# Kolkir/mono_slam_framework

Measured on AMD Instinct MI355X. Metric: frame-pairs/sec (extract+match), higher is better.
Workload: dtype u8; 1 GPU; ORB extract+match, 1280x720 pairs, 1024 pairs/GPU/step resident in HBM, ratio 0.60; pairs_per_gpu=1024, width=1280, height=720, synth_mode=0, overflow_pairs=0, ranks=1, rccl_ranks=0

## Files before the change

mono_slam_framework_amd/csrc/orb_kernels.hip:

```cpp
#include <type_traits>
#include "orb_pipeline.h"

#include <math.h>
#include <stdlib.h>
#include <string.h>

#include "orb_blur_tiles.h"
#include "orb_pattern.h"

namespace msf {

constexpr int SW = TW + 2, SH = TH + 2;
constexpr int kTileCandCap = TW * TH / 4;
constexpr int kTileY0 = kEdge;

constexpr uint32_t kStatusOverflow = 1u;

__constant__ __attribute__((aligned(16))) signed char c_pattern[1024];
__constant__ uint32_t c_disc[2 * kDiscTasks];

__device__ __forceinline__ __amdgpu_buffer_rsrc_t uniform_rsrc(const void* p, uint32_t bytes) {
  const unsigned long long v = (unsigned long long)p;
  const uint32_t lo = (uint32_t)__builtin_amdgcn_readfirstlane((int)(uint32_t)v);
  const uint32_t hi = (uint32_t)__builtin_amdgcn_readfirstlane((int)(uint32_t)(v >> 32));
// ... 1331 lines not shown
                                             int resize_mask, int test_stall_frame, int finish, uint32_t* s1_cnt,
                                             uint4* s1) {
  __shared__ StreamSmem sm;
  const WalkUnit u = walk_unit(g, l_lo, l_hi, n_frames, finish, blockIdx.x);
  if (u.kind == kWalkNone) return;
  const int l = u.level, fi = u.frame, ts = u.strip;
  if (u.kind == kWalkThreshold) {
    if (fi == test_stall_frame && l == 3) return;
    tau_unit(*reinterpret_cast<TauSmem*>(&sm), g, src, pyr, tau, tau_first, redo_cnt, redo_list, qstat, status, abort_word,
             force_tau, predict_pct, chain, l, fi);
    return;
  }
  if (u.kind == kWalkFinish) {
    finish_unit(*reinterpret_cast<FinishSmem*>(&sm), g, src, pyr, tau, tau_first, qstat, cand_cnt, cand_key, cand_sc, cmap,
                redo_cnt, redo_list, s1_cnt, s1, status, abort_word, l, fi);
    return;
  }
  if ((resize_mask >> l) & 1)
    walk_strip<true>(sm, g, src, pyr, tab, qstat, cand_cnt, cand_key, cand_sc, cmap, status, abort_word, margin_pct, dyn, chain, l, fi, ts);
  else
    walk_strip<false>(sm, g, src, pyr, tab, qstat, cand_cnt, cand_key, cand_sc, cmap, status, abort_word, margin_pct, dyn, chain, l, fi, ts);
}

__global__ __launch_bounds__(64) void k_fast_check(OrbGeometry g, int n_frames, uint32_t* tau, uint32_t* tau_first,
                                                   uint32_t* cand_cnt, const uint8_t* cand_sc, const uint2* cmap,
                                                   uint32_t* redo_cnt, uint32_t* redo_list, const uint32_t* qstat) {
  const int fi = blockIdx.x / kOrbLevels, l = blockIdx.x - fi * kOrbLevels, lane = threadIdx.x;
  if (fi >= n_frames || l >= g.nlevels) return;
  const int idx = fi * kOrbLevels + l;
  if (qstat[(size_t)idx * kQStat + kQFin] != 0u) return;
  if (tau[idx] <= (uint32_t)kFastT) return;
  const uint32_t T = max(tau[idx], qstat[(size_t)idx * kQStat + kQTau]);
  const OrbLevelInfo L = g.lv[l];
  const uint2 cm = cmap[idx];
  const bool over = cand_cnt[idx] > cm.y;
  const uint32_t n = min(cand_cnt[idx], cm.y);
  const uint8_t* scs = cand_sc + cm.x;
  const uint32_t found = count_scores_from(scs, n, T, lane);
  if (lane == 0) {
    if (over || found < 2u * (uint32_t)L.quota) {
      tau[idx] = kFastT;
      cand_cnt[idx] = 0;
      redo_list[atomicAdd(redo_cnt, 1u)] = (uint32_t)(fi * kOrbLevels + l);
    } else {
      tau[idx] = T;
      tau_first[idx] = T;
    }
  }
}

__global__ __launch_bounds__(kFastThreads) void k_fast_redo(OrbGeometry g, FrameSrc src, const uint8_t* pyr,
                                                            const uint32_t* __restrict__ redo_cnt,
                                                            const uint32_t* __restrict__ redo_list, int max_tiles,
                                                            uint32_t* cand_cnt, uint32_t* cand_key, uint8_t* cand_sc,
                                                            const uint2* cmap, uint32_t* hist, const uint32_t* emit_thr) {
  __shared__ FastSmem sm;
  const uint32_t n = *redo_cnt;
  const unsigned long long units = (unsigned long long)n * (unsigned)max_tiles;
  const unsigned long long per_xcd = (units + 7ull) >> 3;
  const unsigned long long u_begin = (blockIdx.x & 7u) * per_xcd;
  const unsigned long long u_end = u_begin + per_xcd < units ? u_begin + per_xcd : units;
  for (unsigned long long u = u_begin + (blockIdx.x >> 3); u < u_end; u += (gridDim.x >> 3)) {
    const uint32_t item = redo_list[u / (unsigned)max_tiles];
    const int t = (int)(u % (unsigned)max_tiles);
    const int fi = (int)(item / kOrbLevels), l = (int)(item % kOrbLevels);
    if (t >= g.lv[l].tiles_x * g.lv[l].tiles_y) continue;
    uint32_t emit_min = 0u;
    if (emit_thr) {
      emit_min = emit_thr[item];
      if (emit_min > 255u) continue;
    }
    fast_tile(g, src, pyr, fi, l, t, kFastT, cand_cnt, cand_key, cand_sc, cmap, sm, hist, emit_min);
    __syncthreads();
  }
}

__global__ __launch_bounds__(64) void k_redo_thr(OrbGeometry g, const uint32_t* __restrict__ redo_cnt,
                                                 const uint32_t* __restrict__ redo_list, const uint2* cmap, uint32_t* hist,
                                                 uint32_t* emit_thr) {
  const uint32_t n = *redo_cnt;
  const int lane = threadIdx.x;
  for (uint32_t q = blockIdx.x; q < n; q += gridDim.x) {
    const uint32_t item = redo_list[q];
    const int l = (int)(item % kOrbLevels);
    const int idx = (int)item;
    uint4* const hl = reinterpret_cast<uint4*>(hist + (size_t)idx * 256u);
    const uint4 hv = hl[lane];
    hl[lane] = make_uint4(0u, 0u, 0u, 0u);
    const uint32_t keep = 2u * (uint32_t)g.lv[l].quota;
    uint32_t above = hv.x + hv.y + hv.z + hv.w;
#pragma unroll
    for (int o = 1; o < 64; o <<= 1) {
      const uint32_t up = __shfl_down(above, o);
      if (lane + o < 64) above += up;
    }
    const uint32_t total = __shfl(above, 0);
    above -= hv.x + hv.y + hv.z + hv.w;
    const uint32_t c3 = above + hv.w, c2 = c3 + hv.z, c1 = c2 + hv.y, c0 = c1 + hv.x;
    const int mine = c3 >= keep ? 4 * lane + 3 : c2 >= keep ? 4 * lane + 2 : c1 >= keep ? 4 * lane + 1 : c0 >= keep ? 4 * lane : -1;
    const unsigned long long ok = __ballot(mine >= 0);
    uint32_t thr = 0;
    if (total > keep && total > cmap[idx].y) {
      thr = 256;
      if (keep > 0 && ok) thr = (uint32_t)__shfl(mine, 63 - __builtin_clzll(ok));
    }
    if (lane == 0) emit_thr[idx] = thr;
  }
}

__global__ __launch_bounds__(256) void k_thr_harris(OrbGeometry g, FrameSrc src, const uint8_t* pyr,
                                                    const uint32_t* cand_cnt, const uint32_t* cand_key,
                                                    const uint8_t* cand_sc, const uint2* cmap,
                                                    uint32_t* s1_cnt, uint4* s1, uint32_t* status, int do_harris,
                                                    const uint32_t* fin) {
  __shared__ Stage1Smem S;
  const int l = blockIdx.x, fi = blockIdx.y, tid = threadIdx.x;
  if (l >= g.nlevels) return;
  const int idx = fi * kOrbLevels + l;
  const int slot = src.slot0 + fi;
  if (fin && fin[(size_t)idx * kQStat + kQFin] != 0u) return;
  uint32_t n = cand_cnt[idx];
  const uint2 cm = cmap[idx];
  if (n > cm.y) {
    if (tid == 0) atomicOr(&status[slot], kStatusOverflow);
    n = cm.y;
  }
  stage1_from_list<9>(S, g, src, pyr, l, fi, n, cm, cand_key, cand_sc, s1_cnt, s1, status, do_harris, tid, blockDim.x);
}

__global__ __launch_bounds__(256) void k_harris_flat(OrbGeometry g, FrameSrc src, const uint8_t* pyr, HarrisUnits hw,
                                                     const uint32_t* __restrict__ s1_cnt, uint4* s1,
                                                     const uint32_t* fin) {
  const int fi = blockIdx.y, lane = threadIdx.x & 63;
  const int u = blockIdx.x * 4 + (threadIdx.x >> 6);
  if (u >= hw.base[g.nlevels]) return;
  int l = 0;
#pragma unroll
  for (int i = 1; i < kOrbLevels; i++)
    if (i < g.nlevels && u >= hw.base[i]) l = i;
  if (fin && fin[(size_t)(fi * kOrbLevels + l) * kQStat + kQFin] != 0u) return;
  const OrbLevelInfo L = g.lv[l];
  const uint32_t kept = min(s1_cnt[fi * kOrbLevels + l], (uint32_t)kS1Cap);
  uint4* out = s1 + (long long)fi * g.s1_total + L.s1_off;
  int pitch;
  const uint8_t* img = level_ptr(g, src, pyr, fi, l, &pitch);
  const uint32_t step = 64u * (uint32_t)hw.n[l];
  for (uint32_t i = 64u * (uint32_t)(u - hw.base[l]) + lane; i < kept; i += step) {
    const uint32_t key = out[i].x;
    out[i].y = __float_as_uint(harris_at(img, pitch, key & 0xFFFF, key >> 16));
  }
}

constexpr int kSelCap = kKpCap;
__global__ __launch_bounds__(256) void k_select(OrbGeometry g, int slot0, const uint32_t* s1_cnt, const uint4* s1,
                                                msf_keypoint* kp, uint32_t* kp_cnt, uint32_t* status) {
  __shared__ uint4 kept[kSelCap];
  constexpr int kRespCap = 4096;
  __shared__ __attribute__((aligned(16))) float resp[kRespCap];
  __shared__ __attribute__((aligned(16))) uint32_t keys[kSelCap];
  __shared__ uint32_t nkept;
  const int fi = blockIdx.x, tid = threadIdx.x;
  const int slot = slot0 + fi;
  msf_keypoint* out = kp + (long long)slot * kKpCap;
  uint32_t base = 0;
  bool overflow = false;
  for (int l = 0; l < g.nlevels; l++) {
    const OrbLevelInfo L = g.lv[l];
    const uint32_t n = s1_cnt[fi * kOrbLevels + l];
    const uint4* in = s1 + (long long)fi * g.s1_total + L.s1_off;
    const uint32_t keep = (uint32_t)L.quota;
    if (tid == 0) nkept = 0;
    const bool staged = n > keep && n <= (uint32_t)kRespCap;
    const uint32_t n4 = (n + 3) >> 2;
    if (staged)
      for (uint32_t i = tid; i < 4 * n4; i += 256) resp[i] = i < n ? __uint_as_float(in[i].y) : -INFINITY;
    __syncthreads();
    for (uint32_t i = tid; i < n; i += 256) {
      const uint4 e = in[i];
      bool k = true;
      if (n > keep) {
        const float v = __uint_as_float(e.y);
        uint32_t greater = 0;
        if (staged) {
          const float4* r4 = reinterpret_cast<const float4*>(resp);
          for (uint32_t j = 0; j < n4; j++) {
            const float4 r = r4[j];
            greater += (uint32_t)(r.x > v) + (uint32_t)(r.y > v) + (uint32_t)(r.z > v) + (uint32_t)(r.w > v);
          }
        } else {
          for (uint32_t j = 0; j < n; j++) greater += (__uint_as_float(in[j].y) > v) ? 1u : 0u;
        }
        k = greater < keep;
      }
      if (k) {
        const uint32_t q = atomicAdd(&nkept, 1u);
        if (q < (uint32_t)kSelCap) kept[q] = e;
      }
    }
    __syncthreads();
    uint32_t m = nkept;
    if (m > (uint32_t)kSelCap) { overflow = true; m = kSelCap; }
    if (base + m > (uint32_t)kKpCap) { overflow = true; m = kKpCap - base; }
    const uint32_t m4 = (m + 3) >> 2;
    for (uint32_t i = tid; i < 4 * m4; i += 256) keys[i] = i < m ? kept[i].x : 0xFFFFFFFFu;
    __syncthreads();
    for (uint32_t i = tid; i < m; i += 256) {
      const uint4 e = kept[i];
      uint32_t rank = 0;
      const uint4* k4 = reinterpret_cast<const uint4*>(keys);
      for (uint32_t j = 0; j < m4; j++) {
        const uint4 kk = k4[j];
        rank += (uint32_t)(kk.x < e.x) + (uint32_t)(kk.y < e.x) + (uint32_t)(kk.z < e.x) + (uint32_t)(kk.w < e.x);
      }
      msf_keypoint k;
      k.lx = e.x & 0xFFFF;
      k.ly = e.x >> 16;
      k.x = (float)k.lx * L.scale;
      k.y = (float)k.ly * L.scale;
      k.response = __uint_as_float(e.y);
      k.angle = -1.f;
      k.octave = l;
      k.fast_score = (int)e.z;
      out[base + rank] = k;
    }
    base += m;
    __syncthreads();
  }
  if (tid == 0) {
    kp_cnt[slot] = base;
    if (overflow) atomicOr(&status[slot], kStatusOverflow);
  }
}

__device__ __forceinline__ float fast_atan2_deg(float y, float x) {
  const float k = (float)(180.0 / 3.14159265358979323846);
  const float p1 = 0.9997878412794807f * k, p3 = -0.3258083974640975f * k, p5 = 0.1555786518463281f * k,
              p7 = -0.04432655554792128f * k;
  const float ax = fabsf(x), ay = fabsf(y);
  float a, c, c2;
  if (ax >= ay) {
    c = ay / (ax + (float)2.2204460492503131e-16);
    c2 = c * c;
    a = (((p7 * c2 + p5) * c2 + p3) * c2 + p1) * c;
  } else {
    c = ax / (ay + (float)2.2204460492503131e-16);
    c2 = c * c;
    a = 90.f - (((p7 * c2 + p5) * c2 + p3) * c2 + p1) * c;
  }
  if (x < 0) a = 180.f - a;
  if (y < 0) a = 360.f - a;
  return a;
}

__device__ __forceinline__ void det_sincosf(float t, float* s, float* c) {
  const double x = (double)t;
  const int k = (int)(x * 6.36619772367581382433e-01 + 0.5);
  const double kd = (double)k;
  const double r = (x - kd * 1.57079632673412561417e+00) - kd * 6.07710050650619224932e-11;
  const double z = r * r;
  double p = 1.58969099521155010221e-10;
  p = p * z + -2.50507602534068634195e-08;
  p = p * z + 2.75573137070700676789e-06;
  p = p * z + -1.98412698298579493134e-04;
  p = p * z + 8.33333333332248946124e-03;
  p = p * z + -1.66666666666666324348e-01;
  const double sr = r + (r * z) * p;
  double q = -1.13596475577881948265e-11;
  q = q * z + 2.08757232129817482790e-09;
  q = q * z + -2.75573143513906633035e-07;
  q = q * z + 2.48015872894767294178e-05;
  q = q * z + -1.38888888888741095749e-03;
  q = q * z + 4.16666666666666019037e-02;
  const double cr = (1.0 - 0.5 * z) + (z * z) * q;
  double sv, cv;
  switch (k & 3) {
    case 0: sv = sr; cv = cr; break;
    case 1: sv = cr; cv = -sr; break;
    case 2: sv = -sr; cv = -cr; break;
    default: sv = -cr; cv = sr; break;
  }
  *s = (float)sv;
  *c = (float)cv;
}

constexpr int PR = 22;
constexpr int PD = 2 * PR + 1;
constexpr int PP = blur_tiles::kRawPitch;
constexpr int HP = blur_tiles::kHbCols;
constexpr int HC = blur_tiles::kHbPitch;
static_assert(PD == blur_tiles::kRawRows && PD * (PP / 4) == blur_tiles::kFetchLoads * blur_tiles::kFetchLanes, "patch fetch");
typedef int v4i_t __attribute__((ext_vector_type(4)));

template <bool HALF_UP, bool SUM256>
__global__ __launch_bounds__(256) void k_describe(OrbGeometry g, FrameSrc src, const uint8_t* pyr,
                                                  msf_keypoint* kp, const uint32_t* kp_cnt, uint8_t* desc) {
  __shared__ __attribute__((aligned(16))) uint8_t raw_s[4][blur_tiles::kRawBytes];
  __shared__ __attribute__((aligned(16))) uint16_t hb_s[4][blur_tiles::kHbEntries];
  __shared__ uint32_t disc_s[2 * kDiscTasks];
  __shared__ __attribute__((aligned(16))) int pat_s[256];
  int fi = blockIdx.y, part = blockIdx.x;
  if (gridDim.x == 8 && (fi | 7) < (int)gridDim.y) {
    part = fi & 7;
    fi = (fi & ~7) | (int)blockIdx.x;
  }
  const int slot = src.slot0 + fi;
  const int wave = __builtin_amdgcn_readfirstlane((int)(threadIdx.x >> 6)), lane = threadIdx.x & 63;
  for (int i = threadIdx.x; i < 2 * kDiscTasks; i += 256) disc_s[i] = c_disc[i];
  pat_s[threadIdx.x] = reinterpret_cast<const int*>(c_pattern)[threadIdx.x];
  __shared__ unsigned long long lvl_base_s[kOrbLevels];
  __shared__ int lvl_pitch_s[kOrbLevels];
  if (threadIdx.x < kOrbLevels) {
    int pt = 0;
    const uint8_t* bp = level_ptr(g, src, pyr, fi, threadIdx.x < g.nlevels ? (int)threadIdx.x : 0, &pt);
    lvl_base_s[threadIdx.x] = (unsigned long long)bp;
    lvl_pitch_s[threadIdx.x] = pt;
  }
  __syncthreads();
  const uint32_t count = min(kp_cnt[slot], (uint32_t)kKpCap);
  uint8_t* raw = raw_s[wave];
  uint16_t* hb = hb_s[wave];
  uint32_t* raw32 = reinterpret_cast<uint32_t*>(raw);
  constexpr int NPL = blur_tiles::kFetchLoads;
  const uint32_t kstride = gridDim.x * 4;
  uint32_t k = (uint32_t)part * 4 + wave;
  uint32_t pre[NPL];
  auto meta = [&](uint32_t k_) -> uint3 {
    if (k_ >= count) return make_uint3(0u, 0u, 0u);
    const msf_keypoint* Kp = kp + (long long)slot * kKpCap + k_;
    return make_uint3((uint32_t)Kp->octave, (uint32_t)Kp->lx, (uint32_t)Kp->ly);
  };
  const int fl = blur_tiles::fetch_lane(lane);
  const uint32_t fetch_row = (uint32_t)blur_tiles::fetch_row(lane), fetch_x4 = 4u * (uint32_t)blur_tiles::fetch_dword(lane);
  auto issue = [&](uint3 m) {
    const uint32_t lv = (uint32_t)__builtin_amdgcn_readfirstlane((int)m.x);
    const int mx = __builtin_amdgcn_readfirstlane((int)m.y), my = __builtin_amdgcn_readfirstlane((int)m.z);
    const uint32_t pitch_ = (uint32_t)__builtin_amdgcn_readfirstlane(lvl_pitch_s[lv]);
    const unsigned long long b64 = lvl_base_s[lv];
    const unsigned long long img_ = ((unsigned long long)(uint32_t)__builtin_amdgcn_readfirstlane((int)(b64 >> 32)) << 32) |
                                    (uint32_t)__builtin_amdgcn_readfirstlane((int)(uint32_t)b64);
    typedef const __attribute__((address_space(1))) uint8_t* gptr_t;
    const unsigned long long base = img_ + (unsigned long long)((long long)(my - PR) * (long long)pitch_ + (mx - PP / 2));
    const uint32_t off = mad_u24(fetch_row, pitch_, fetch_x4);
#pragma unroll
    for (int u = 0; u < NPL; u++)
      pre[u] = *(const __attribute__((address_space(1))) uint32_t*)((gptr_t)(base + (unsigned long long)(5u * (uint32_t)u * pitch_)) + off);
  };
  const uint32_t raw_lds = (uint32_t)(uintptr_t)(__attribute__((address_space(3))) uint8_t*)raw;
  const uint32_t hb_lds = (uint32_t)(uintptr_t)(__attribute__((address_space(3))) uint16_t*)hb;
  const uint32_t blur_a = (uint32_t)blur_tiles::a_byte_offset(0, lane);
  const uint32_t blur_w = (uint32_t)blur_tiles::hb_store_byte_offset(0, 0, lane);
  v4i_t blur_b[blur_tiles::kTilesN];
#pragma unroll
  for (int nt = 0; nt < blur_tiles::kTilesN; nt++)
#pragma unroll
    for (int d = 0; d < 4; d++) blur_b[nt][d] = (int)blur_tiles::b_dword(SUM256, nt, lane, d);
  const bool blur_cols = (lane & 15) < HP - 32;
  const bool blur_rows = (lane >> 4) < 3;
  static_assert(blur_tiles::kSampleReach == PR - 3, "the blur's three taps on either side of the pattern's reach");
  const uint32_t samp_base = hb_lds + (uint32_t)blur_tiles::samp_byte_offset(0, 0) - 2u * HC * 0x400000u - 2u * 0x4B400000u;
  uint3 m_cur = meta(k), m_next = meta(k + kstride);
  if (k < count) issue(m_cur);
  for (; k < count; k += kstride) {
    const bool active = true;
    msf_keypoint* K = kp + (long long)slot * kKpCap + k;
    const int l = (int)m_cur.x, cx = (int)m_cur.y, cy = (int)m_cur.z;
    (void)l; (void)cx; (void)cy;
#pragma unroll
    for (int u = 0; u < NPL; u++) raw32[60 * u + fl] = pre[u] ^ 0x80808080u;
    m_cur = m_next;
    if (k + kstride < count) issue(m_cur);
    m_next = meta(k + 2 * kstride);
    MSF_WAVE_SYNC();
    float angle = 0.f;
    if (active) {
      int m10 = 0, m01 = 0;
      {
#pragma unroll
        for (int it = 0; it < kDiscTasks / 64; it++) {
          const int t = it * 64 + lane;
          const int row = t >> 3, k = t & 7;
          const uint32_t pxw = raw32[(row + 7) * (PP / 4) + 2 + k];
// ... 330 lines not shown
  MSF_HIP_TRY(d_redo_thr_.reserve(Wk * kOrbLevels * sizeof(uint32_t)));
  MSF_HIP_TRY(d_qstat_.reserve(Wk * kOrbLevels * kQStat * sizeof(uint32_t)));
  MSF_HIP_TRY(hipMemset(d_qstat_, 0, Wk * kOrbLevels * kQStat * sizeof(uint32_t)));
  MSF_HIP_TRY(d_cand_.reserve(total * sizeof(uint32_t)));
  MSF_HIP_TRY(d_cand_sc_.reserve(total));
  MSF_HIP_TRY(d_cmap_.reserve(Wk * kOrbLevels * sizeof(uint2)));
  MSF_HIP_TRY(hipMemset(d_cmap_, 0, Wk * kOrbLevels * sizeof(uint2)));
  MSF_HIP_TRY(d_walk_abort_.reserve(16));
  MSF_HIP_TRY(hipMemset(d_walk_abort_, 0, 16));
  MSF_HIP_TRY(hipHostMalloc(&h_walk_abort_, 16, hipHostMallocDefault));
  h_walk_abort_[0] = h_walk_abort_[1] = 0u;
  MSF_HIP_TRY(d_s1_cnt_.reserve(Wk * kOrbLevels * sizeof(uint32_t)));
  MSF_HIP_TRY(d_s1_.reserve(Wk * g.s1_total * sizeof(uint4)));
  MSF_HIP_TRY(d_kp_.reserve(S * kKpCap * sizeof(msf_keypoint)));
  MSF_HIP_TRY(d_desc_.reserve(S * kKpCap * 32));
  MSF_HIP_TRY(d_kp_cnt_.reserve(S * sizeof(uint32_t)));
  MSF_HIP_TRY(d_status_.reserve(S * sizeof(uint32_t)));
  MSF_HIP_TRY(d_qres_.reserve((size_t)kSplitMaxPairs * kKpCap * sizeof(uint32_t)));
  MSF_HIP_TRY(d_done_.reserve((size_t)kSplitMaxPairs * sizeof(uint32_t)));
  MSF_HIP_TRY(hipMemset(d_done_, 0, (size_t)kSplitMaxPairs * sizeof(uint32_t)));
  MSF_HIP_TRY(hipMemset(d_kp_cnt_, 0, S * sizeof(uint32_t)));
  MSF_HIP_TRY(hipMemset(d_status_, 0, S * sizeof(uint32_t)));
  MSF_HIP_TRY(hipMemset(d_cand_cnt_, 0, Wk * kOrbLevels * sizeof(uint32_t)));
  MSF_HIP_TRY(hipMemset(d_s1_cnt_, 0, Wk * kOrbLevels * sizeof(uint32_t)));
  MSF_HIP_TRY(hipMemcpyToSymbol(HIP_SYMBOL(c_pattern), k_orb_bit_pattern_31, 1024));
  MSF_HIP_TRY(hipMemcpyToSymbol(HIP_SYMBOL(c_disc), plan.disc.data(), sizeof(uint32_t) * 2 * kDiscTasks));
  if (profile_) {
    for (auto& set : evr_)
      for (auto& e : set.ev) MSF_HIP_TRY(hipEventCreate(&e));
    ev_ok_ = true;
  }
  return "";
}

__global__ __launch_bounds__(256) void k_fill_u32(uint32_t* a, uint32_t* b, uint32_t v, int n) {
  const int i = blockIdx.x * 256 + threadIdx.x;
  if (i < n) { a[i] = v; b[i] = v; }
}

hipError_t OrbPipeline::extract(const FrameSrc& src, int n, hipStream_t st) {
  if (n <= 0) return hipSuccess;
  if (src.slot0 < 0 || src.slot0 + n > max_slots_ || n > work_frames_) return hipErrorInvalidValue;
  last_src_ = src;
  last_n_ = n;
  if (h_walk_abort_ && !walk_per_level_ && __atomic_load_n(&h_walk_abort_[1], __ATOMIC_RELAXED) != 0u) {
    walk_per_level_ = true;
    degraded_note_ = true;
  }
  if (test_stall_frame_ >= 0 && test_stall_calls_++ > 0) test_stall_frame_ = -1;
  if (ev_ok_) ev_begin_call();
  const hipError_t e = extract_range(src, n, st, ev_ok_ ? ev_ : nullptr);
  if (ev_ok_) ev_extract_pending_ = true;
  return e;
}

hipError_t OrbPipeline::extract_range(const FrameSrc& src, int n, hipStream_t st, hipEvent_t* evs) {
  const OrbGeometry& g = g_;
  hipError_t e;
  if ((e = hipMemsetAsync(d_cand_cnt_, 0, (size_t)n * kOrbLevels * 4, st))) return e;
  if ((e = hipMemsetAsync(d_status_ + src.slot0, 0, (size_t)n * 4, st))) return e;
  if ((e = hipMemsetAsync(d_redo_, 0, 4, st))) return e;
  if (evs) hipEventRecord(evs[0], st);
  uint32_t* const tau = d_tau_;
  uint32_t* const tau_first = d_tau_ + (size_t)work_frames_ * kOrbLevels;
  const int force_tau = call_force_tau(n);
  const bool dense = force_tau == kFastT;
  if (dense && (long long)n * g.cand_total > (long long)g.pool_entries) return hipErrorInvalidValue;
  hipLaunchKernelGGL(k_cand_reset, dim3((n * kOrbLevels + 255) / 256), dim3(256), 0, st, g, prim_, d_cmap_, n, dense ? 1 : 0);
  const int dyn = (fast_two_part_ && force_tau == 0) ? 1 : 0;
  bool fused = fused_ && !dense && g.total_tiles > 0;
  for (int l = 1; l < g.nlevels; l++) fused = fused && g.lv[l].wk_fused != 0;
  auto launch_walk = [&](int l_lo, int l_hi, int chain, int resize_mask, int predict_pct, int finish) {
    const long long wgs = walk_grid(g, l_lo, l_hi, n, finish);
    hipLaunchKernelGGL(k_walk, dim3((unsigned)wgs), dim3(64), 0, st, g, src, d_pyr_, d_tab_, tau, tau_first, d_qstat_,
                       d_cand_cnt_, d_cand_, d_cand_sc_, d_cmap_, d_redo_, d_redo_ + 1, d_status_, d_walk_abort_, l_lo, l_hi, n,
                       tau2_margin_pct_, dyn, force_tau, predict_pct, chain, resize_mask, test_stall_frame_, finish,
                       d_s1_cnt_, d_s1_);
  };
  last_fused_ = fused;
  last_dense_ = dense;
  last_finish_ = false;
  if (!dense && g.total_tiles > 0) {
    if ((e = hipMemsetAsync(d_qstat_, 0, (size_t)n * kOrbLevels * kQStat * 4, st))) return e;
    if ((e = hipMemsetAsync(d_walk_abort_, 0, 4, st))) return e;
  }
  if (fused) {
    const int mask = (1 << (g.nlevels - 1)) - 1;
    const int predict = dyn ? tau_predict_pct_ : 0;
    if (walk_per_level_) {
      for (int l = 0; l < g.nlevels; l++) launch_walk(l, l, 1, mask, predict, kWalkFinishOff);
    } else {
      launch_walk(0, g.nlevels - 1, 1, mask, predict, walk_finish_);
      last_finish_ = walk_finish_ != kWalkFinishOff;
    }
    hipMemcpyAsync(h_walk_abort_, d_walk_abort_, 8, hipMemcpyDeviceToHost, st);
    if (evs) hipEventRecord(evs[1], st);
  } else {
    for (int l = 1; l < g.nlevels; l++) launch_resize(src, n, l, st);
    if (evs) hipEventRecord(evs[1], st);
    if (g.total_tiles > 0) {
      if (dense) {
        hipLaunchKernelGGL(k_fill_u32, dim3((n * kOrbLevels + 255) / 256), dim3(256), 0, st, tau, tau_first,
                           (uint32_t)kFastT, n * kOrbLevels);
        hipLaunchKernelGGL(k_fast, dim3((unsigned)g.total_tiles * (unsigned)n), dim3(kFastThreads), 0, st, g, src, d_pyr_,
                           d_cand_cnt_, d_cand_, d_cand_sc_, d_cmap_);
      } else {
        launch_walk(0, g.nlevels - 1, 0, 0, 0, kWalkFinishOff);
      }
    }
  }
  if (g.total_tiles > 0 && !dense) {
    hipLaunchKernelGGL(k_fast_check, dim3((unsigned)n * kOrbLevels), dim3(64), 0, st, g, n, tau, tau_first,
                       d_cand_cnt_, d_cand_sc_, d_cmap_, d_redo_, d_redo_ + 1, d_qstat_);
    long long units = (long long)n * kOrbLevels * g.max_level_tiles;
    unsigned grid = (unsigned)(units < 2048 ? units : 2048);
    grid = (grid + 7u) & ~7u;
    hipLaunchKernelGGL(k_fast_redo, dim3(grid), dim3(kFastThreads), 0, st, g, src, d_pyr_, d_redo_, d_redo_ + 1,
                       g.max_level_tiles, d_cand_cnt_, d_cand_, d_cand_sc_, d_cmap_, d_redo_hist_, (const uint32_t*)nullptr);
    hipLaunchKernelGGL(k_redo_thr, dim3((unsigned)std::min<long long>((long long)n * kOrbLevels, 1024)), dim3(64), 0, st, g,
                       d_redo_, d_redo_ + 1, d_cmap_, d_redo_hist_, d_redo_thr_);
    hipLaunchKernelGGL(k_fast_redo, dim3(grid), dim3(kFastThreads), 0, st, g, src, d_pyr_, d_redo_, d_redo_ + 1,
                       g.max_level_tiles, d_cand_cnt_, d_cand_, d_cand_sc_, d_cmap_, (uint32_t*)nullptr, d_redo_thr_);
  }
  if (evs) hipEventRecord(evs[2], st);
  launch_tail(src, n, dense, st, evs, !dense && g.total_tiles > 0 ? d_qstat_ : nullptr);
  return hipGetLastError();
}

void OrbPipeline::launch_resize(const FrameSrc& src, int n, int l, hipStream_t st) {
  const OrbGeometry& g = g_;
  const OrbLevelInfo& L = g.lv[l];
  const int sw16 = (g.lv[l - 1].w + 16 + 15) & ~15;
  const int groups = (L.w + 3) >> 2;
  int rth = 8;
  const int threads = 256;
  while (rth > 4 && ((rth * 5 + 3) / 4 + 3) * sw16 > 60000) rth -= 4;
  const int lds_rows = (rth * 5 + 3) / 4 + 3;
  const uint32_t magic_n16 = (uint32_t)(0x100000000ull / (uint32_t)(sw16 >> 4)) + 1u;
  const uint32_t magic_groups = groups > 1 ? (uint32_t)(0x100000000ull / (uint32_t)groups) + 1u : 0u;
  hipLaunchKernelGGL(resize_shared_[l] ? k_resize<true> : k_resize<false>, dim3((L.h + rth - 1) / rth, n), dim3(threads),
                     (size_t)lds_rows * sw16 + 8 * kResizeMaxRows, st, g, src, d_pyr_, d_tab_, l, rth, lds_rows, magic_n16,
                     magic_groups);
}

void OrbPipeline::launch_tail(const FrameSrc& src, int n, bool dense, hipStream_t st, hipEvent_t* evs, const uint32_t* fin) {
  const OrbGeometry& g = g_;
  hipLaunchKernelGGL(k_thr_harris, dim3(g.nlevels, n), dim3(dense ? 256 : 64), 0, st, g, src, d_pyr_,
                     d_cand_cnt_, d_cand_, d_cand_sc_, d_cmap_, d_s1_cnt_, d_s1_, d_status_, dense ? 1 : 0, fin);
  if (!dense) {
    const HarrisUnits& hw = harris_;
    const int nu = hw.base[kOrbLevels];
    hipLaunchKernelGGL(k_harris_flat, dim3((nu + 3) / 4, n), dim3(256), 0, st, g, src, d_pyr_, hw, d_s1_cnt_, d_s1_, fin);
  }
  hipLaunchKernelGGL(k_select, dim3(n), dim3(256), 0, st, g, src.slot0, d_s1_cnt_, d_s1_, d_kp_, d_kp_cnt_,
                     d_status_);
  if (evs) hipEventRecord(evs[3], st);
  {
    int bx = 2048 / n;
    bx = bx < 8 ? 8 : bx > 128 ? 128 : bx;
    auto kd = blur_sum256_ ? k_describe<true, true> : half_up_ ? k_describe<true, false> : k_describe<false, false>;
    hipLaunchKernelGGL(kd, dim3(bx, n), dim3(256), 0, st, g, src, d_pyr_, d_kp_, d_kp_cnt_, d_desc_);
  }
  if (evs) hipEventRecord(evs[4], st);
}

std::string OrbPipeline::tail_refusal(int n, const int32_t* counts, const int32_t* cands) const {
  if (n < 1 || n > work_frames_) return "n_frames outside [1, 2*max_batch_pairs]";
  const bool dense = call_force_tau(n) == kFastT;
  int cap[kOrbLevels];
  for (int l = 0; l < kOrbLevels; l++) cap[l] = l < g_.nlevels ? (dense ? g_.lv[l].cand_cap : prim_.cap[l]) : 0;
  return check_tail_lists(g_, cap, n, counts, cands);
}

hipError_t OrbPipeline::tail(const FrameSrc& src, int n, const int32_t* counts, const int32_t* cands, int form,
                             hipStream_t st) {
  if (n <= 0) return hipSuccess;
  if (src.slot0 < 0 || src.slot0 + n > max_slots_ || n > work_frames_) return hipErrorInvalidValue;
  const OrbGeometry& g = g_;
  const bool dense = call_force_tau(n) == kFastT;
  if (dense && (long long)n * g.cand_total > (long long)g.pool_entries) return hipErrorInvalidValue;
  last_src_ = src;
  last_n_ = n;
  last_fused_ = false;
  last_dense_ = true;
  hipError_t e;
  if ((e = hipMemsetAsync(d_status_ + src.slot0, 0, (size_t)n * 4, st))) return e;
  hipLaunchKernelGGL(k_cand_reset, dim3((n * kOrbLevels + 255) / 256), dim3(256), 0, st, g, prim_, d_cmap_, n, dense ? 1 : 0);
  hipLaunchKernelGGL(k_fill_u32, dim3((n * kOrbLevels + 255) / 256), dim3(256), 0, st, d_tau_,
                     d_tau_ + (size_t)work_frames_ * kOrbLevels, (uint32_t)kFastT, n * kOrbLevels);
  for (int l = 1; l < g.nlevels; l++) launch_resize(src, n, l, st);
  std::vector<uint2> cmap((size_t)n * kOrbLevels);
  if ((e = hipMemcpyAsync(cmap.data(), d_cmap_, cmap.size() * sizeof(uint2), hipMemcpyDeviceToHost, st))) return e;
  if ((e = hipStreamSynchronize(st))) return e;
  size_t total = 0;
  for (int i = 0; i < n * kOrbLevels; i++) total += (size_t)counts[i];
  std::vector<uint32_t> keys(total ? total : 1), cnt((size_t)n * kOrbLevels);
  std::vector<uint8_t> scs(total ? total : 1);
  for (size_t i = 0; i < total; i++) {
    keys[i] = (uint32_t)cands[3 * i] | (uint32_t)cands[3 * i + 1] << 16;
    scs[i] = (uint8_t)cands[3 * i + 2];
  }
  size_t off = 0;
  for (int i = 0; i < n * kOrbLevels; i++) {
    cnt[i] = (uint32_t)counts[i];
    const size_t m = std::min<size_t>(cnt[i], cmap[i].y);
    if (m) {
      if ((e = hipMemcpyAsync(d_cand_ + (size_t)cmap[i].x, keys.data() + off, m * 4, hipMemcpyHostToDevice, st))) break;
      if ((e = hipMemcpyAsync(d_cand_sc_ + (size_t)cmap[i].x, scs.data() + off, m, hipMemcpyHostToDevice, st))) break;
    }
    off += cnt[i];
  }
  if (!e) e = hipMemcpyAsync(d_cand_cnt_, cnt.data(), cnt.size() * 4, hipMemcpyHostToDevice, st);
  if (!e) {
    launch_tail(src, n, form == 0, st, nullptr, nullptr);
    e = hipGetLastError();
  }
  const hipError_t es = hipStreamSynchronize(st);
  return e ? e : es;
}

static int train_chunk() {
  static const int chunk = [] {
    const char* e = getenv("MSF_ORB_TRAIN_CHUNK");
    const int v = e ? atoi(e) : kTrainChunk;
    return v >= 16 && v <= kTrainChunk ? v : kTrainChunk;
  }();
  return chunk;
}

hipError_t OrbPipeline::set_features(int slot, int n, const msf_keypoint* kp, const uint8_t* desc, hipStream_t st) {
  hipError_t e = hipSuccess;
  if (n > 0) {
    e = hipMemcpyAsync(d_kp_ + (size_t)slot * kKpCap, kp, (size_t)n * sizeof(msf_keypoint), hipMemcpyHostToDevice, st);
    if (e != hipSuccess) return e;
    e = hipMemcpyAsync(d_desc_ + (size_t)slot * kKpCap * 32, desc, (size_t)n * 32, hipMemcpyHostToDevice, st);
    if (e != hipSuccess) return e;
  }
  set_words_[0] = (uint32_t)n;
  set_words_[1] = 0u;
  e = hipMemcpyAsync(d_kp_cnt_ + slot, &set_words_[0], sizeof(uint32_t), hipMemcpyHostToDevice, st);
  if (e != hipSuccess) return e;
  return hipMemcpyAsync(d_status_ + slot, &set_words_[1], sizeof(uint32_t), hipMemcpyHostToDevice, st);
}

hipError_t OrbPipeline::match(int n_pairs, const int32_t* d_slot_a, const int32_t* d_slot_b, float ratio,
                              msf_match* d_out, int cap, int32_t* d_n_out, hipStream_t st, int slot_base, int slot_limit) {
  if (n_pairs <= 0) return hipSuccess;
  const int limit = slot_limit > 0 && slot_limit < max_slots_ ? slot_limit : max_slots_;
  if (ev_ok_ && !ev_extract_pending_) {
    ev_begin_call();
    hipEventRecord(ev_[4], st);
  }
  const int chunk = train_chunk();
  const bool split = n_pairs <= kSplitMaxPairs && d_qres_;
  last_match_form_ = split ? 1 : 2;
  if (split)
    hipLaunchKernelGGL(k_match_split, dim3(kSplitBlocks, n_pairs), dim3(256), 0, st, n_pairs, d_slot_a, d_slot_b, d_kp_,
                       d_kp_cnt_, d_desc_, d_status_, ratio, d_out, cap, d_n_out, chunk, d_qres_, d_done_, slot_base, limit);
  else
    hipLaunchKernelGGL(k_match, dim3(n_pairs), dim3(256), 0, st, n_pairs, d_slot_a, d_slot_b, d_kp_, d_kp_cnt_,
                       d_desc_, d_status_, ratio, d_out, cap, d_n_out, chunk, slot_base, limit);
  if (ev_ok_) {
    hipEventRecord(ev_[5], st);
    EvSet& set = evr_[ev_cur_];
    set.recorded = true;
    set.match_only = !ev_extract_pending_;
    ev_extract_pending_ = false;
  }
  return hipGetLastError();
}

void OrbPipeline::ev_begin_call() {
  if (evr_[ev_cur_].recorded) {
    ev_cur_ = (ev_cur_ + 1) % kEvRing;
    if (evr_[ev_cur_].recorded) ev_harvest(ev_cur_);
  }
  ev_ = evr_[ev_cur_].ev;
}

void OrbPipeline::ev_harvest(int i) {
  EvSet& set = evr_[i];
  if (!set.recorded) return;
  set.recorded = false;
  if (hipEventSynchronize(set.ev[5]) != hipSuccess) return;
  for (int k = set.match_only ? 4 : 0; k < 5; k++) {
    float t = 0.f;
    if (hipEventElapsedTime(&t, set.ev[k], set.ev[k + 1]) == hipSuccess) acc_ms_[k] += t;
  }
  if (set.match_only) acc_match_only_++;
  else acc_full_++;
}

int OrbPipeline::stage_times(const char** names, float* ms, int cap) {
  const char* kNames[5] = {last_fused_ ? "pyramid_fast" : "pyramid", "fast_nms", "select_harris", "orient_describe", "match"};
  if (!ev_ok_) return 0;
  for (int k = 0; k < kEvRing; k++) ev_harvest((ev_cur_ + 1 + k) % kEvRing);
  if (acc_full_ + acc_match_only_ == 0) return 0;
  int n = 0;
  for (int i = acc_full_ ? 0 : 4; i < 5 && n < cap; i++, n++) {
    names[n] = kNames[i];
    ms[n] = acc_ms_[i];
  }
  for (auto& a : acc_ms_) a = 0.f;
  acc_full_ = acc_match_only_ = 0;
  return n;
}

// ... 162 lines not shown
```

Baseline: 170,700 frame-pairs/sec.

## Rewrite keypoint selection as per-level wave radix threshold search

```diff
diff --git a/mono_slam_framework_amd/csrc/orb_kernels.hip b/mono_slam_framework_amd/csrc/orb_kernels.hip
--- a/mono_slam_framework_amd/csrc/orb_kernels.hip
+++ b/mono_slam_framework_amd/csrc/orb_kernels.hip
@@ -1507,81 +1507,165 @@
 }
 
 constexpr int kSelCap = kKpCap;
-__global__ __launch_bounds__(256) void k_select(OrbGeometry g, int slot0, const uint32_t* s1_cnt, const uint4* s1,
-                                                msf_keypoint* kp, uint32_t* kp_cnt, uint32_t* status) {
-  __shared__ uint4 kept[kSelCap];
-  constexpr int kRespCap = 4096;
-  __shared__ __attribute__((aligned(16))) float resp[kRespCap];
-  __shared__ __attribute__((aligned(16))) uint32_t keys[kSelCap];
-  __shared__ uint32_t nkept;
-  const int fi = blockIdx.x, tid = threadIdx.x;
+constexpr int kSelStage = 512;
+constexpr int kSelPer = kSelStage / 64;
+struct SelectSmem {
+  uint32_t keys[kOrbLevels][kSelStage];
+  uint32_t resp[kOrbLevels][kSelStage];
+  uint8_t score[kOrbLevels][kSelStage];
+  uint32_t total[kOrbLevels];
+};
+
+__device__ __forceinline__ uint32_t select_ord(uint32_t bits) {
+  if (bits == 0x80000000u) bits = 0u;
+  return bits ^ ((bits >> 31) ? 0xFFFFFFFFu : 0x80000000u);
+}
+
+template <typename F>
+__device__ __forceinline__ void select_for_nk(const uint32_t nk, F&& f) {
+  static_assert(kSelPer == 8, "one case per entry a lane may hold");
+  switch (nk) {
+    case 1: f(std::integral_constant<int, 1>{}); break;
+    case 2: f(std::integral_constant<int, 2>{}); break;
+    case 3: f(std::integral_constant<int, 3>{}); break;
+    case 4: f(std::integral_constant<int, 4>{}); break;
+    case 5: f(std::integral_constant<int, 5>{}); break;
+    case 6: f(std::integral_constant<int, 6>{}); break;
+    case 7: f(std::integral_constant<int, 7>{}); break;
+    default: f(std::integral_constant<int, 8>{}); break;
+  }
+}
+
+__device__ __forceinline__ void select_store(msf_keypoint* at, const uint32_t key, const uint32_t resp, const uint32_t score,
+                                             const float scale, const int l) {
+  msf_keypoint k;
+  k.lx = key & 0xFFFF;
+  k.ly = key >> 16;
+  k.x = (float)k.lx * scale;
+  k.y = (float)k.ly * scale;
+  k.response = __uint_as_float(resp);
+  k.angle = -1.f;
+  k.octave = l;
+  k.fast_score = (int)score;
+  *at = k;
+}
+
+__global__ __launch_bounds__(64 * kOrbLevels) __attribute__((amdgpu_waves_per_eu(8, 8))) void k_select(
+    OrbGeometry g, int slot0, const uint32_t* s1_cnt, const uint4* s1, msf_keypoint* kp, uint32_t* kp_cnt, uint32_t* status) {
+  __shared__ __attribute__((aligned(16))) SelectSmem S;
+  static_assert(kOrbLevels == 8, "the pairing of levels on a SIMD");
+  const int w = threadIdx.x >> 6, lane = threadIdx.x & 63;
+  const int l = w < 4 ? w : 11 - w;
+  const int fi = blockIdx.x;
   const int slot = slot0 + fi;
-  msf_keypoint* out = kp + (long long)slot * kKpCap;
-  uint32_t base = 0;
+  uint32_t n = 0, keep = 0, total = 0;
+  float scale = 0.f;
+  const uint4* in = s1;
+  if (l < g.nlevels) {
+    n = min(s1_cnt[fi * kOrbLevels + l], (uint32_t)kS1Cap);
+    keep = (uint32_t)g.lv[l].quota;
+    scale = g.lv[l].scale;
+    in = s1 + (long long)fi * g.s1_total + g.lv[l].s1_off;
+  }
+  const bool staged = n <= (uint32_t)kSelStage;
+  uint32_t cut = 0;
+  const bool none = n > keep && keep == 0u;
+  uint32_t ex[kSelPer], ey[kSelPer], rank[kSelPer];
+  if (staged) {
+    uint32_t ez[kSelPer / 4] = {};
+#pragma unroll
+    for (int k = 0; k < kSelPer; k++) {
+      const uint32_t i = lane + 64u * k;
+      const uint4 e = i < n ? in[i] : make_uint4(0u, 0u, 0u, 0u);
+      ex[k] = e.x, ey[k] = e.y, ez[k >> 2] |= (e.z & 255u) << (8 * (k & 3));
+      rank[k] = i < n ? select_ord(e.y) : 0u;
+    }
+    if (n > keep && keep > 0u)
+      select_for_nk((n + 63u) >> 6, [&](auto nk) {
+        for (int b = 31; b >= 0; b--) {
+          const uint32_t c = cut | (1u << b);
+          uint32_t cnt = 0;
+#pragma unroll
+          for (int k = 0; k < nk; k++) cnt += (uint32_t)__popcll(__ballot(rank[k] >= c));
+          if (cnt >= keep) cut = c;
+        }
+      });
+#pragma unroll
+    for (int k = 0; k < kSelPer; k++) {
+      const bool kept = lane + 64u * k < n && !none && rank[k] >= cut;
+      const unsigned long long b = __ballot(kept);
+      if (kept) {
+        const uint32_t at = total + (uint32_t)__popcll(b & ((1ull << lane) - 1ull));
+        S.keys[l][at] = ex[k], S.resp[l][at] = ey[k], S.score[l][at] = (uint8_t)(ez[k >> 2] >> (8 * (k & 3)));
+      }
+      total += (uint32_t)__popcll(b);
+    }
+    const uint32_t t4 = (total + 3u) >> 2;
+    if ((uint32_t)lane < 4u * t4 - total) S.keys[l][total + lane] = 0xFFFFFFFFu;
+    MSF_WAVE_SYNC();
+#pragma unroll
+    for (int k = 0; k < kSelPer; k++) {
+      ex[k] = lane + 64u * k < total ? S.keys[l][lane + 64u * k] : 0xFFFFFFFFu;
+      rank[k] = 0;
+    }
+    if (total)
+      select_for_nk((total + 63u) >> 6, [&](auto nk) {
+        const uint4* k4 = reinterpret_cast<const uint4*>(S.keys[l]);
+        for (uint32_t j = 0; j < t4; j++) {
+          const uint4 s = k4[j];
+#pragma unroll
+          for (int k = 0; k < nk; k++)
+            rank[k] += (uint32_t)(s.x < ex[k]) + (uint32_t)(s.y < ex[k]) + (uint32_t)(s.z < ex[k]) + (uint32_t)(s.w < ex[k]);
+        }
+      });
+  } else {
+    if (n > keep && keep > 0u)
+      for (int b = 31; b >= 0; b--) {
+        const uint32_t c = cut | (1u << b);
+        uint32_t cnt = 0;
+        for (uint32_t i0 = 0; i0 < n; i0 += 64u)
+          cnt += (uint32_t)__popcll(__ballot(i0 + lane < n && select_ord(in[min(i0 + lane, n - 1u)].y) >= c));
+        if (cnt >= keep) cut = c;
+      }
+    for (uint32_t i0 = 0; i0 < n; i0 += 64u)
+      total += (uint32_t)__popcll(__ballot(i0 + lane < n && !none && select_ord(in[min(i0 + lane, n - 1u)].y) >= cut));
+  }
+  if (lane == 0) S.total[l] = total;
+  __syncthreads();
+  uint32_t base = 0, my_base = 0, my_m = 0;
   bool overflow = false;
-  for (int l = 0; l < g.nlevels; l++) {
-    const OrbLevelInfo L = g.lv[l];
-    const uint32_t n = s1_cnt[fi * kOrbLevels + l];
-    const uint4* in = s1 + (long long)fi * g.s1_total + L.s1_off;
-    const uint32_t keep = (uint32_t)L.quota;
-    if (tid == 0) nkept = 0;
-    const bool staged = n > keep && n <= (uint32_t)kRespCap;
-    const uint32_t n4 = (n + 3) >> 2;
-    if (staged)
-      for (uint32_t i = tid; i < 4 * n4; i += 256) resp[i] = i < n ? __uint_as_float(in[i].y) : -INFINITY;
-    __syncthreads();
-    for (uint32_t i = tid; i < n; i += 256) {
-      const uint4 e = in[i];
-      bool k = true;
-      if (n > keep) {
-        const float v = __uint_as_float(e.y);
-        uint32_t greater = 0;
-        if (staged) {
-          const float4* r4 = reinterpret_cast<const float4*>(resp);
-          for (uint32_t j = 0; j < n4; j++) {
-            const float4 r = r4[j];
-            greater += (uint32_t)(r.x > v) + (uint32_t)(r.y > v) + (uint32_t)(r.z > v) + (uint32_t)(r.w > v);
-          }
-        } else {
-          for (uint32_t j = 0; j < n; j++) greater += (__uint_as_float(in[j].y) > v) ? 1u : 0u;
-        }
-        k = greater < keep;
-      }
-      if (k) {
-        const uint32_t q = atomicAdd(&nkept, 1u);
-        if (q < (uint32_t)kSelCap) kept[q] = e;
-      }
-    }
-    __syncthreads();
-    uint32_t m = nkept;
+  for (int j = 0; j < g.nlevels; j++) {
+    uint32_t m = S.total[j];
     if (m > (uint32_t)kSelCap) { overflow = true; m = kSelCap; }
     if (base + m > (uint32_t)kKpCap) { overflow = true; m = kKpCap - base; }
-    const uint32_t m4 = (m + 3) >> 2;
-    for (uint32_t i = tid; i < 4 * m4; i += 256) keys[i] = i < m ? kept[i].x : 0xFFFFFFFFu;
-    __syncthreads();
-    for (uint32_t i = tid; i < m; i += 256) {
-      const uint4 e = kept[i];
-      uint32_t rank = 0;
-      const uint4* k4 = reinterpret_cast<const uint4*>(keys);
-      for (uint32_t j = 0; j < m4; j++) {
-        const uint4 kk = k4[j];
-        rank += (uint32_t)(kk.x < e.x) + (uint32_t)(kk.y < e.x) + (uint32_t)(kk.z < e.x) + (uint32_t)(kk.w < e.x);
-      }
-      msf_keypoint k;
-      k.lx = e.x & 0xFFFF;
-      k.ly = e.x >> 16;
-      k.x = (float)k.lx * L.scale;
-      k.y = (float)k.ly * L.scale;
-      k.response = __uint_as_float(e.y);
-      k.angle = -1.f;
-      k.octave = l;
-      k.fast_score = (int)e.z;
-      out[base + rank] = k;
-    }
+    if (j == l) my_base = base, my_m = m;
     base += m;
-    __syncthreads();
-  }
-  if (tid == 0) {
+  }
+  msf_keypoint* out = kp + (long long)slot * kKpCap + my_base;
+  if (staged) {
+#pragma unroll
+    for (int k = 0; k < kSelPer; k++) {
+      const uint32_t i = lane + 64u * k;
+      if (i < total && rank[k] < my_m) select_store(out + rank[k], ex[k], S.resp[l][i], S.score[l][i], scale, l);
+    }
+  } else {
+    for (uint32_t i0 = 0; i0 < n && my_m; i0 += 64u) {
+      const uint32_t i = i0 + lane;
+      const uint4 e = in[min(i, n - 1u)];
+      const bool kept = i < n && !none && select_ord(e.y) >= cut;
+      if (__ballot(kept) == 0ull) continue;
+      uint32_t r = 0;
+      for (uint32_t j0 = 0; j0 < n; j0 += 64u) {
+        const uint32_t j = j0 + lane;
+        const uint4 ej = in[min(j, n - 1u)];
+        const uint32_t kj = j < n && !none && select_ord(ej.y) >= cut ? ej.x : 0xFFFFFFFFu;
+#pragma unroll
+        for (int jj = 0; jj < 64; jj++) r += (uint32_t)((uint32_t)__builtin_amdgcn_readlane((int)kj, jj) < e.x);
+      }
+      if (kept && r < my_m) select_store(out + r, e.x, e.y, e.z, scale, l);
+    }
+  }
+  if (threadIdx.x == 0) {
     kp_cnt[slot] = base;
     if (overflow) atomicOr(&status[slot], kStatusOverflow);
   }
@@ -2218,7 +2302,7 @@
     const int nu = hw.base[kOrbLevels];
     hipLaunchKernelGGL(k_harris_flat, dim3((nu + 3) / 4, n), dim3(256), 0, st, g, src, d_pyr_, hw, d_s1_cnt_, d_s1_, fin);
   }
-  hipLaunchKernelGGL(k_select, dim3(n), dim3(256), 0, st, g, src.slot0, d_s1_cnt_, d_s1_, d_kp_, d_kp_cnt_,
+  hipLaunchKernelGGL(k_select, dim3(n), dim3(64 * kOrbLevels), 0, st, g, src.slot0, d_s1_cnt_, d_s1_, d_kp_, d_kp_cnt_,
                      d_status_);
   if (evs) hipEventRecord(evs[3], st);
   {
```

Measured after the change: 173,600 frame-pairs/sec (median of 3 runs). About the same (+1.7%).
